# atharris/basilisk_env

Measured on NVIDIA B200. Metric: env decision-steps/sec, higher is better.
Workload: dtype f64

## Files before the change

basilisk_env_b200/csrc/leo_core.cuh:

```cuda
#pragma once
#include <math.h>
#include <stdint.h>
#include "leo_params.h"

#if defined(__CUDACC__)
#define LEO_HD __host__ __device__ __forceinline__
#define LEO_HD_NOINLINE static __host__ __device__ __noinline__
#else
#define LEO_HD inline
#define LEO_HD_NOINLINE static inline
#endif

#ifndef LEO_UNROLL_STAGES
#define LEO_UNROLL_STAGES 0
#endif

namespace leo {

struct V3 { double x, y, z; };
struct M3 { V3 a, b, c; };
LEO_HD V3 mk(double x, double y, double z) { V3 v; v.x = x; v.y = y; v.z = z; return v; }
LEO_HD V3 operator+(V3 p, V3 q) { return mk(p.x + q.x, p.y + q.y, p.z + q.z); }
LEO_HD V3 operator-(V3 p, V3 q) { return mk(p.x - q.x, p.y - q.y, p.z - q.z); }
LEO_HD V3 operator-(V3 p) { return mk(-p.x, -p.y, -p.z); }
// ... 767 lines not shown
        if (desat_quiet) {
            const int64_t cnt = I[(int64_t)I_DUMPCNT * stride + e];
            I[(int64_t)I_DUMPCNT * stride + e] = cnt <= 0 ? (int64_t)P.maxCounterValue : cnt - 1;
            I[(int64_t)I_DUMPPRIOR * stride + e] = now_ns;
            desat_ran = 4;
        } else {
            desat_ran = 1 | (fsw_desat<NRW>(P, S, I, stride, e, now_ns, ws) << 1);
        }
    }
    if (mask & LEO_TASK_MRP) {
        AttGuid g;
        g.sigma_BR = mld3(m, M_GUID); g.omega_BR_B = mld3(m, M_GUID + 3);
        g.omega_RN_B = mld3(m, M_GUID + 6); g.domega_RN_B = mld3(m, M_GUID + 9);
        V3 Lr = mrp_feedback(P, g);
        mst3(m, M_LR, Lr);
        g = att_tracking_error(ns, nw, ref);
        mst3(m, M_GUID, g.sigma_BR); mst3(m, M_GUID + 3, g.omega_BR_B);
        mst3(m, M_GUID + 6, g.omega_RN_B); mst3(m, M_GUID + 9, g.domega_RN_B);
        V3 mLr = -Lr;
#pragma unroll
        for (int i = 0; i < NRW; i++) mst(m, M_RWCMD + i, P.Umap[i][0] * mLr.x + P.Umap[i][1] * mLr.y + P.Umap[i][2] * mLr.z);
    }
    return desat_ran;
}

LEO_HD V3 add_cross(V3 p, V3 u, V3 v)
{
    return mk(fmad(u.y, v.z, fmad(-u.z, v.y, p.x)), fmad(u.z, v.x, fmad(-u.x, v.z, p.y)), fmad(u.x, v.y, fmad(-u.y, v.x, p.z)));
}
LEO_HD V3 sub_cross(V3 p, V3 u, V3 v)
{
    return mk(fmad(-u.y, v.z, fmad(u.z, v.y, p.x)), fmad(-u.z, v.x, fmad(u.x, v.z, p.y)), fmad(-u.x, v.y, fmad(u.y, v.x, p.z)));
}

LEO_HD V3 sun_accel(const LeoParams &P, V3 rs, V3 r)
{
    V3 d = r - rs;
    double is = rsq(dot(rs, rs)), id = rsq(dot(d, d));
    return rs * (-P.mu_sun * (is * is * is)) + d * (-P.mu_sun * (id * id * id));
}

LEO_HD V3 sun_window(const LeoParams &P, MBus m, const Dyn &x, double dt0, double h_first, int w, double dyn_s)
{
    const double half = 0.5 * (h_first + (double)(w - 1) * dyn_s);
    return sun_accel(P, mld3(m, M_SUNR) + mld3(m, M_SUNV) * (dt0 + half), x.r + x.v * half);
}

struct StageIn {
    V3 Lc;
    V3 gsun;
    V3 HB, tau_u;
    double rho, h;
    double dtp;
};

template <int J2, bool DIAG>
LEO_HD void eom(const LeoParams &P, const Dyn &x, Dyn &k, const StageIn &a, double ct, bool thr_on, MBus m)
{
    V3 g;
    {
        double ir = rsq(dot(x.r, x.r));
        double ir3 = ir * ir * ir;
        g = a.gsun + x.r * (-P.mu_c * ir3);
        if (J2 == 2) {
            const V3 D0 = mld3(m, M_PFIX) + mld3(m, M_PFIXD) * a.dtp;
            const V3 D1 = mld3(m, M_PFIX + 3) + mld3(m, M_PFIXD + 3) * a.dtp;
            const V3 D2 = mld3(m, M_PFIX + 6) + mld3(m, M_PFIXD + 6) * a.dtp;
            const V3 rp = mk(dot(D0, x.r), dot(D1, x.r), dot(D2, x.r));
            const double ip = rsq(dot(rp, rp)), ip2 = ip * ip, ip5 = ip2 * ip2 * ip;
            const V3 Mr = mk(P.gm2[0] * rp.x + P.gm2[3] * rp.y + P.gm2[4] * rp.z,
                             P.gm2[3] * rp.x + P.gm2[1] * rp.y + P.gm2[5] * rp.z,
                             P.gm2[4] * rp.x + P.gm2[5] * rp.y + P.gm2[2] * rp.z);
            const double q5 = -5. * dot(rp, Mr) * ip5 * ip2;
            const V3 gp = Mr * (2. * ip5) + rp * q5;
            g = g + D0 * gp.x + D1 * gp.y + D2 * gp.z;
        } else if (J2) {
            double ir2 = ir * ir, z2 = 5. * x.r.z * x.r.z * ir2, kk = -P.j2k * ir3 * ir2;
            g = g + mk(kk * x.r.x * (1. - z2), kk * x.r.y * (1. - z2), kk * x.r.z * (3. - z2));
        }
    }
    MrpRot R = mrp_rot(x.s);
    V3 vB = rot_BN(R, x.s, x.v);
    V3 Mp;
    double Sp;
    {
        double ax = fabs(vB.x), ay = fabs(vB.y), az = fabs(vB.z);
        Sp = P.dragKa[0] * ax + P.dragKa[1] * ay + P.dragKa[2] * az;
        if (!DIAG) Sp += P.dragKd[0] * vB.x + P.dragKd[1] * vB.y + P.dragKd[2] * vB.z;
        if (DIAG) {
            Mp = mk(P.dragMa[0][0] * ax + P.dragMd[0][0] * vB.x, P.dragMa[1][1] * ay + P.dragMd[1][1] * vB.y,
                    P.dragMa[2][2] * az + P.dragMd[2][2] * vB.z);
        } else {
            Mp = arr(P.dragMa[0]) * ax + arr(P.dragMa[1]) * ay + arr(P.dragMa[2]) * az
               + arr(P.dragMd[0]) * vB.x + arr(P.dragMd[1]) * vB.y + arr(P.dragMd[2]) * vB.z;
        }
    }
    const double mrho = -a.rho;
    k.v = g + x.v * (mrho * Sp);
    if (thr_on) k.v = k.v + rot_NB(R, x.s, mld3(m, M_FM));
    k.r = x.v;
    V3 rot = add_cross(a.Lc, Mp * mrho, vB);
    const V3 hw = a.HB + a.tau_u * ct;
    if (DIAG) {
        V3 h = mk(fmad(P.D[0], x.w.x, hw.x), fmad(P.D[4], x.w.y, hw.y), fmad(P.D[8], x.w.z, hw.z));
        rot = sub_cross(rot, x.w, h);
        k.w = mk(rot.x * P.Dinv[0], rot.y * P.Dinv[4], rot.z * P.Dinv[8]);
    } else {
        V3 h = mv9(P.D, x.w) + hw;
        rot = sub_cross(rot, x.w, h);
        k.w = mv9(P.Dinv, rot);
    }
    {
        double sw = dot(x.s, x.w);
        k.s = x.w * (0.25 * R.oms2) + cross(x.s, x.w) * 0.5 + x.s * (0.5 * sw);
    }
}

template <int J2, bool DIAG>
LEO_HD Dyn rk4_step(const LeoParams &P, const Dyn &x, const StageIn &a, bool thr_on, MBus m)
{
    const double h = a.h, hh = 0.5 * h, h6 = h * (1.0 / 6.0), h3 = h * (1.0 / 3.0);
    Dyn k, acc;
    k.r = k.v = k.s = k.w = acc.r = acc.v = acc.s = acc.w = mk(0., 0., 0.);
    double c = 0.;
#if LEO_UNROLL_STAGES == 2
#pragma unroll 2
#elif LEO_UNROLL_STAGES
#pragma unroll
#else
#pragma unroll 1
#endif
    for (int st = 0; st < 4; st++) {
        Dyn xs;
        xs.r = x.r + k.r * c; xs.v = x.v + k.v * c; xs.s = x.s + k.s * c; xs.w = x.w + k.w * c;
        eom<J2, DIAG>(P, xs, k, a, c, thr_on, m);
        const double wo = (st == 0 || st == 3) ? h6 : h3;
        acc.r = acc.r + k.r * wo; acc.v = acc.v + k.v * wo; acc.s = acc.s + k.s * wo; acc.w = acc.w + k.w * wo;
        c = (st == 2) ? h : hh;
    }
    Dyn xo;
    xo.r = x.r + acc.r; xo.v = x.v + acc.v; xo.s = x.s + acc.s; xo.w = x.w + acc.w;
    return xo;
}

struct SunDt { double d0, dm, d1; };
struct ThrEventOut { Dyn x; int factor, active; };
template <int J2, bool DIAG>
LEO_HD_NOINLINE ThrEventOut rk4_general(const LeoParams &P, const double *S, int64_t stride, int64_t e, MBus m, Dyn x,
                                        StageIn a, SunDt dts, double tBefore, double tauPrev, int thr_factor, int thr_active)
{
    const double h = a.h, hh = 0.5 * h, h6 = h * (1.0 / 6.0), h3 = h * (1.0 / 3.0);
    const V3 sun_r = mld3(m, M_SUNR), sun_v = mld3(m, M_SUNV), L_ext = mld3(m, M_LEXT);
    Dyn xs = x, xo = x, k;
    ThrCmd tc = {};
    if (thr_active) tc = thr_cmd_load(S, stride, e);
#pragma unroll 1
    for (int st = 0; st < 4; st++) {
        const double dt = (st == 0) ? dts.d0 : (st == 3 ? dts.d1 : dts.dm);
        const double ct = (st == 0) ? 0.0 : (st == 3 ? h : hh);
        a.gsun = sun_accel(P, sun_r + sun_v * dt, xs.r);
        a.dtp = dt;
        V3 Fm = mk(0., 0., 0.), Lx = L_ext;
        const bool thr_on = thr_active != 0;
        if (thr_on) {
            const double tau = t_add(tBefore, (st == 0) ? 0.0 : (st == 3 ? h : t_mul(h, 0.5)));
            ThrOut to = thr_stage(P, tc, tau, t_sub(tau, tauPrev), thr_factor);
            thr_factor = to.factor; thr_active = to.active;
            Fm = to.F * P.inv_mass; Lx = Lx + to.L;
            tauPrev = tau;
        }
        a.Lc = Lx - a.tau_u;
        mst3(m, M_FM, Fm);
        eom<J2, DIAG>(P, xs, k, a, ct, thr_on, m);
        const double wo = (st == 0 || st == 3) ? h6 : h3;
        const double cn = (st == 2) ? h : hh;
        xo.r = xo.r + k.r * wo; xo.v = xo.v + k.v * wo; xo.s = xo.s + k.s * wo; xo.w = xo.w + k.w * wo;
        if (st < 3) { xs.r = x.r + k.r * cn; xs.v = x.v + k.v * cn; xs.s = x.s + k.s * cn; xs.w = x.w + k.w * cn; }
    }
    ThrEventOut o;
    o.x = xo; o.factor = thr_factor; o.active = thr_active;
    return o;
}

struct ThrRefresh { V3 Lc, L_thr; double t_next; };
LEO_HD_NOINLINE ThrRefresh thr_refresh(const LeoParams &P, const double *S, int64_t stride, int64_t e, MBus m, int factor, V3 tau_u)
{
    ThrRefresh o;
    V3 F = mk(0., 0., 0.);
    o.L_thr = mk(0., 0., 0.); o.t_next = 1e300;
    double start = S[(int64_t)F_THRSTART * stride + e];
    for (int k = 0; k < LEO_NTHR; k++) {
        if (!((factor >> k) & 1)) continue;
        V3 f = arr(P.thr_dir[k]) * (P.thr_Fmax * 1.0);
        F = f + F;
        o.L_thr = cross(arr(P.thr_loc[k]), f) + o.L_thr;
        double t_off = t_add(S[(int64_t)(F_THRON + k) * stride + e], start);
        if (t_off < o.t_next) o.t_next = t_off;
    }
    mst3(m, M_FM, F * P.inv_mass);
    o.Lc = (mld3(m, M_LEXT) + o.L_thr) - tau_u;
    return o;
}

LEO_HD_NOINLINE SunDt sun_dt_wrapped(double prev_ns_d, double sun_ns_d, double tBefore, double prevTime, double h)
{
    SunDt o;
    uint64_t sun_ns = (uint64_t)sun_ns_d;
    uint64_t s0 = (uint64_t)t_add(prev_ns_d, t_div(t_sub(tBefore, prevTime), 1e-9));
    uint64_t sm = (uint64_t)t_add(prev_ns_d, t_div(t_sub(t_add(tBefore, t_mul(h, 0.5)), prevTime), 1e-9));
    uint64_t s1 = (uint64_t)t_add(prev_ns_d, t_div(t_sub(t_add(tBefore, h), prevTime), 1e-9));
    o.d0 = t_mul((double)(s0 - sun_ns), 1e-9);
    o.dm = t_mul((double)(sm - sun_ns), 1e-9);
    o.d1 = t_mul((double)(s1 - sun_ns), 1e-9);
    return o;
}

template <int NRW>
struct PostOut { double uJ[NRW]; V3 Lc, tau_u; int thr_active, quiet; };
template <int NRW>
LEO_HD void wheel_latch(const LeoParams &P, MBus m, const double (&W)[NRW], V3 L_thr, double (&uJ)[NRW], V3 &Lc, V3 &tau_u_out)
{
    V3 tau_u = mk(0., 0., 0.);
#pragma unroll
    for (int i = 0; i < NRW; i++) {
        double uc = mld(m, M_RWCMD + i);
        if (P.u_max[i] > 0.) { if (uc > P.u_max[i]) uc = P.u_max[i]; else if (uc < -P.u_max[i]) uc = -P.u_max[i]; }
        if (fabs(uc) < P.u_min[i]) uc = 0.0;
        if (fabs(W[i]) >= P.Om_max[i] && P.Om_max[i] > 0.0 && W[i] * uc >= 0.0) uc = 0.0;
        mst(m, M_U + i, uc);
        uJ[i] = uc * P.invJs[i];
        tau_u = tau_u + arr(P.gs[i]) * uc;
    }
    tau_u_out = tau_u;
    Lc = (mld3(m, M_LEXT) + L_thr) - tau_u;
}
template <int NRW>
LEO_HD_NOINLINE PostOut<NRW> post_tick_events(const LeoParams &P, double *S, int64_t *I, int64_t stride, int64_t e, MBus m,
                                              const double (&W)[NRW], V3 L_thr, int desat_ran, int64_t now_ns, int thr_factor)
{
    PostOut<NRW> o;
    wheel_latch<NRW>(P, m, W, L_thr, o.uJ, o.Lc, o.tau_u);
    o.thr_active = -1; o.quiet = 0;
    if (desat_ran & 1) {
        o.thr_active = thr_latch(P, S, I, stride, e, now_ns, thr_factor);
        o.quiet = (desat_ran & 2) && o.thr_active == 0;
    } else if (desat_ran & 4) {
        S[(int64_t)F_THRSTART * stride + e] = t_mul((double)now_ns, 1.0E-9);
        o.quiet = 1;
    }
    return o;
}

#define LEO_THR_MARGIN 1e-6

template <int NRW, bool DIAG>
LEO_HD void wheel_speeds(const LeoParams &P, V3 HB, const double (&C)[NRW], V3 w, double (&W)[NRW])
{
    if (DIAG) {
        W[0] = fmad(HB.x, P.invJs[0], -w.x); W[1] = fmad(HB.y, P.invJs[1], -w.y); W[2] = fmad(HB.z, P.invJs[2], -w.z);
    } else {
#pragma unroll
        for (int i = 0; i < NRW; i++) W[i] = C[i] - dot(arr(P.gs[i]), w);
    }
}

#if defined(__CUDACC__)
__constant__ double LEO_K[16] = {
    1.4426950408889634, 6755399441055744.0, -6.93147180369123816490e-01, -1.90821492927058770002e-10,
    1. / 6., 1. / 24., 1. / 120., 1. / 720., 1. / 5040., 1. / 40320., 1. / 362880., 1. / 3628800., 1. / 39916800.,
    1. / 479001600., 1. / 6227020800.,
    1e-9};
#endif
#if defined(__CUDA_ARCH__)
#define LEO_NANO2SEC LEO_K[15]
#else
#define LEO_NANO2SEC 1e-9
#endif
LEO_HD double exp_bounded(double x)
{
#ifdef __CUDA_ARCH__
    x = fmin(fmax(x, -700.0), 700.0);
    const double t = fma(x, LEO_K[0], LEO_K[1]);
    const int kk = __double2loint(t);
    const double kd = t - LEO_K[1];
    double r = fma(kd, LEO_K[2], x);
    r = fma(kd, LEO_K[3], r);
    const double r2 = r * r, r4 = r2 * r2, r8 = r4 * r4;
    const double a0 = r + 1.0, a1 = fma(r, LEO_K[4], 0.5), a2 = fma(r, LEO_K[6], LEO_K[5]), a3 = fma(r, LEO_K[8], LEO_K[7]);
    const double a4 = fma(r, LEO_K[10], LEO_K[9]), a5 = fma(r, LEO_K[12], LEO_K[11]);
    const double a6 = fma(r, LEO_K[14], LEO_K[13]);
    const double b0 = fma(a1, r2, a0), b1 = fma(a3, r2, a2), b2 = fma(a5, r2, a4);
    const double d0 = fma(b1, r4, b0), d1 = fma(a6, r4, b2);
    const double p = fma(d1, r8, d0);
    return __hiloint2double(__double2hiint(p) + (kk << 20), __double2loint(p));
#else
    return exp(x);
#endif
}

}
#include "leo_f32.cuh"
namespace leo {

template <int NRW, int J2, bool DIAG, bool F32 = false>
LEO_HD void leo_step_env(const LeoParams &P, double *__restrict__ S, int64_t *__restrict__ I, int64_t stride, int64_t e,
                         MBus m, int action, StepOut &out, const LeoParamsF &PF = LeoParamsF(), int chunk = 0, int n_chunks = 1)
{
#define SD(f) S[(int64_t)(f) * stride + e]
#define SI(f) I[(int64_t)(f) * stride + e]
    Dyn x;
    StageIn a;
    x.r = mk(SD(F_R), SD(F_R + 1), SD(F_R + 2));
    x.v = mk(SD(F_V), SD(F_V + 1), SD(F_V + 2));
    x.s = mk(SD(F_SIG), SD(F_SIG + 1), SD(F_SIG + 2));
    x.w = mk(SD(F_OMG), SD(F_OMG + 1), SD(F_OMG + 2));
    double C[NRW], uJ[NRW];
    a.tau_u = mk(0., 0., 0.); a.HB = mk(0., 0., 0.);
#pragma unroll
    for (int i = 0; i < NRW; i++) {
        const double u = SD(F_UCUR + i);
        mst(m, M_U + i, u);
        uJ[i] = u * P.invJs[i];
        C[i] = SD(F_WHL + i) + dot(arr(P.gs[i]), x.w);
        a.tau_u = a.tau_u + arr(P.gs[i]) * u;
        a.HB = a.HB + arr(P.gs[i]) * (P.Js[i] * C[i]);
    }
    for (int f = 0; f < LEO_M_MIRROR; f++) mst(m, f, SD(F_GUID + f));
    a.rho = SD(F_RHO);
    {
        const V3 L_ext = mk(SD(F_LDIST), SD(F_LDIST + 1), SD(F_LDIST + 2));
        mst3(m, M_LEXT, L_ext); mst3(m, M_FM, mk(0., 0., 0.));
        a.Lc = L_ext - a.tau_u;
    }
    mst3(m, M_LTHR, mk(0., 0., 0.));
    const int64_t tick = SI(I_TICK);
    int mask = (int)SI(I_MASK);
    int thr_factor = (int)SI(I_THRFACTOR), thr_active = (int)SI(I_THRACTIVE), rw_sat = (int)SI(I_RWSAT);
    int nswitch = 0;

    if (chunk > 0) {}
    else if (action == 0) mask = LEO_TASK_NADIR | LEO_TASK_MRP;
    else if (action == 1) mask = LEO_TASK_SUN | LEO_TASK_MRP;
    else if (action == 2) {
        mask = LEO_TASK_SUN | LEO_TASK_MRP | LEO_TASK_DESAT;
        SI(I_INITREQ) = 1;
        SI(I_DUMPPRIOR) = 0; SI(I_DUMPCNT) = 0; SI(I_LASTDH) = 0;
        for (int k = 0; k < LEO_NTHR; k++) SD(F_THRREM + k) = 0.0;
    }
    mst(m, M_TNEXT, -1.0);

    const bool first = tick < 0;
    const int tpf = P.ticks_per_fsw;
    const int ticks_step = tpf * P.fsw_per_step;
    const int ticks = ticks_step / n_chunks;
    const int64_t n_base = (first ? 0 : tick) + 1;
    const int64_t n_step0 = ((n_base - 1) / ticks_step) * ticks_step;
    const int64_t n_end = n_step0 + ticks_step;
    const double dyn_d = (double)P.dyn_ns;
    double sun_d = (double)(n_step0 * P.dyn_ns);
    sun_latch_to_bus(P, m, n_step0 * P.dyn_ns);
    if (J2 == 2) pfix_latch_to_bus(P, m, n_step0 * P.dyn_ns);
    a.dtp = 0.;
    V3f sunr_f = mkf(0.f, 0.f, 0.f), sunv_f = mkf(0.f, 0.f, 0.f);
    float ecf[6] = {0.f, 0.f, 0.f, 0.f, 0.f, 0.f};
    if (F32) {
        sunr_f = tof(mld3(m, M_SUNR)); sunv_f = tof(mld3(m, M_SUNV));
#pragma unroll
        for (int q = 0; q < 6; q++) ecf[q] = (float)mld(m, M_ECL + q);
    }
    const int j0 = first ? -1 : 0;
    int phase = (int)((n_base + j0) % tpf);
    double now_d = (double)((n_base + j0) * P.dyn_ns);
    int desat_ran = 0, desat_quiet = 0;
    double charge = SD(F_E), shadow = SD(F_SHADOW);
    double newTime = t_mul(now_d, LEO_NANO2SEC);
    double prevTime = j0 < 0 ? 0.0 : t_mul(now_d - dyn_d, 1e-9);
    double h = t_sub(newTime, prevTime);
    double dtsm = t_mul((j0 < 0 ? 0.0 : now_d - dyn_d) - sun_d, LEO_NANO2SEC) + 0.5 * h;
    const double dyn_s = t_mul(dyn_d, LEO_NANO2SEC);
    if (!F32) a.gsun = sun_window(P, m, x, dtsm - 0.5 * h, h, tpf - phase, dyn_s);

#pragma unroll 1
    for (int j = j0; j < ticks; j++) {
        bool wrapped = false;
        if (LEO_RARE(phase == 0)) {
            const int64_t n = n_base + j;
            double W[NRW];
            wheel_speeds<NRW, DIAG>(P, a.HB, C, x.w, W);
#ifndef LEO_EXP_NOFSW
            desat_ran = fsw_pass<NRW>(P, S, I, stride, e, m, mask, n, n * P.dyn_ns, x, W, (int64_t)sun_d, desat_quiet);
            rw_sat |= 2;
#endif
            if (n > 0 && n == n_end) {
                sun_d = now_d; sun_latch_to_bus(P, m, n * P.dyn_ns); wrapped = true;
                if (J2 == 2) pfix_latch_to_bus(P, m, n * P.dyn_ns);
                if (F32) {
                    sunr_f = tof(mld3(m, M_SUNR)); sunv_f = tof(mld3(m, M_SUNV));
#pragma unroll
                    for (int q = 0; q < 6; q++) ecf[q] = (float)mld(m, M_ECL + q);
                }
            }
            if (!F32) a.gsun = sun_window(P, m, x, t_mul((j < 0 ? 0.0 : now_d - dyn_d) - sun_d, LEO_NANO2SEC), h, tpf, dyn_s);
        }
        a.h = h;
        if (LEO_RARE(wrapped || (thr_active && !(newTime + LEO_THR_MARGIN <= mld(m, M_TNEXT))))) {
            const double prev_d = j < 0 ? 0.0 : now_d - dyn_d;
            const double tBefore = t_sub(newTime, h);
            SunDt dts;
            dts.d0 = t_mul(prev_d - sun_d, 1e-9); dts.dm = dts.d0 + 0.5 * h; dts.d1 = dts.d0 + h;
            if (wrapped) dts = sun_dt_wrapped(prev_d, sun_d, tBefore, prevTime, h);
            double tauPrev = 0.0;
            if (j >= 0) {
                const double ppT = (n_base + j > 1) ? t_mul(prev_d - dyn_d, 1e-9) : 0.0;
                const double ph = t_sub(prevTime, ppT);
                tauPrev = t_add(t_sub(prevTime, ph), ph);
            }
            ThrEventOut o = rk4_general<J2, DIAG>(P, S, stride, e, m, x, a, dts, tBefore, tauPrev, thr_factor, thr_active);
            x = o.x; thr_factor = o.factor; thr_active = o.active;
            ThrRefresh th = thr_refresh(P, S, stride, e, m, thr_active ? thr_factor : 0, a.tau_u);
            a.Lc = th.Lc; mst3(m, M_LTHR, th.L_thr); mst(m, M_TNEXT, th.t_next);
        } else if (F32) {
            StageInF af;
            af.h = (float)h; af.rho = (float)a.rho;
            af.Lc = tof(a.Lc); af.HB = tof(a.HB); af.tau_u = tof(a.tau_u);
            af.gsun = sun_accelf(PF, sunr_f + sunv_f * (float)dtsm, tof(x.r) + tof(x.v) * (0.5f * af.h));
            const bool thr_on = thr_active != 0;
            x = rk4_step_mixed<(J2 != 0), DIAG>(PF, x, af, thr_on, thr_on ? tof(mld3(m, M_FM)) : mkf(0.f, 0.f, 0.f));
        } else {
            if (J2 == 2) a.dtp = dtsm;
            x = rk4_step<J2, DIAG>(P, x, a, thr_active != 0, m);
        }
        a.HB = a.HB + a.tau_u * h;
        if (!DIAG) {
#pragma unroll
            for (int i = 0; i < NRW; i++) C[i] = fmad(uJ[i], h, C[i]);
        }
        {
            const double s2 = dot(x.s, x.s);
            const bool sw = s2 > 1.0000000000000002;
            const double f = -frcp(sw ? s2 : 1.0);
            x.s = mk(sw ? x.s.x * f : x.s.x, sw ? x.s.y * f : x.s.y, sw ? x.s.z * f : x.s.z);
            nswitch += sw ? 1 : 0;
        }
        double r2 = 0., ir = 0., id = 0., rdh = 0., pgeo = 0.;
        bool penumbra = false;
        float shf = 0.f, panel_f = 0.f;
        V3f xr_f = mkf(0.f, 0.f, 0.f);
        if (F32) {
            xr_f = tof(x.r);
            const float r2f = dot(xr_f, xr_f);
            a.rho = (double)(PF.rho0 * expf(-(r2f * rsqf(r2f) - PF.Rp_atmo) * PF.inv_H));
            const V3f r_SBf = sunr_f - xr_f;
            const float d2f = dot(r_SBf, r_SBf), idf = rsqf(d2f);
            shf = eclipse_coref(PF, ecf, sunr_f, xr_f, r2f, d2f);
            penumbra = shf < 0.f;
            const V3f sf = tof(x.s);
            MrpRotF R = mrp_rotf(sf);
            V3f n_N = rot_NBf(R, sf, arrf(PF.nHat_B));
            float proj = dot(n_N, r_SBf) * idf;
            if (proj < 0.f) proj = 0.f;
            panel_f = PF.panel_coef * proj * (idf * idf);
        } else {
            r2 = dot(x.r, x.r); ir = rsq(r2);
            a.rho = P.rho0 * exp_bounded(-(r2 * ir - P.Rp_atmo) * P.inv_H);
        }
        double W[NRW];
        wheel_speeds<NRW, DIAG>(P, a.HB, C, x.w, W);
        int lim = 0;
#pragma unroll
        for (int i = 0; i < NRW; i++) lim |= (fabs(W[i]) >= P.Om_max[i] && P.Om_max[i] > 0.0) ? 1 : 0;
#ifndef LEO_EXP_NOENV
        if (!F32) {
            const V3 sun_r = mld3(m, M_SUNR);
            const V3 r_SB = sun_r - x.r;
            const double d2 = dot(r_SB, r_SB);
            id = rsq(d2);
            const double ec[6] = {mld(m, M_ECL), mld(m, M_ECL + 1), mld(m, M_ECL + 2), mld(m, M_ECL + 3), mld(m, M_ECL + 4), mld(m, M_ECL + 5)};
            shadow = eclipse_cones(P, ec, sun_r, x.r, r2, d2, penumbra);
            rdh = dot(x.r, r_SB);
            MrpRot R = mrp_rot(x.s);
            V3 n_N = rot_NB(R, x.s, arr(P.nHat_B));
            double proj = dot(n_N, r_SB) * id;
            if (proj < 0.) proj = 0.;
            pgeo = P.panel_coef * proj * (id * id);
        }
#endif
        const double h_this = h;
        now_d += dyn_d;
        phase = (phase + 1 == tpf) ? 0 : phase + 1;
        prevTime = newTime;
        newTime = t_mul(now_d, LEO_NANO2SEC);
        h = t_sub(newTime, prevTime);
        dtsm = t_mul((now_d - dyn_d) - sun_d, LEO_NANO2SEC) + 0.5 * h;
        if (LEO_RARE(rw_sat | lim | desat_ran)) {
            PostOut<NRW> po = post_tick_events<NRW>(P, S, I, stride, e, m, W, mld3(m, M_LTHR), desat_ran, (int64_t)(now_d - dyn_d), thr_factor);
#pragma unroll
            for (int i = 0; i < NRW; i++) uJ[i] = po.uJ[i];
            a.Lc = po.Lc; a.tau_u = po.tau_u;
            rw_sat = lim;
            if (po.thr_active >= 0) { thr_active = po.thr_active; mst(m, M_TNEXT, -1.0); }
            if (desat_ran) desat_quiet = po.quiet;
            desat_ran = 0;
        }
        if (LEO_RARE(penumbra)) {
            if (F32) {
                const V3 sun_r = mld3(m, M_SUNR);
                const V3 r_SB = sun_r - x.r;
                const double r2d = dot(x.r, x.r), d2 = dot(r_SB, r_SB);
                const double ec[6] = {mld(m, M_ECL), mld(m, M_ECL + 1), mld(m, M_ECL + 2), mld(m, M_ECL + 3), mld(m, M_ECL + 4), mld(m, M_ECL + 5)};
                shadow = eclipse_core(P, ec, sun_r, x.r, r2d, rsq(r2d), r_SB, d2, rsq(d2));
                shf = (float)shadow;
            } else {
#ifdef LEO_LITERAL_ECLIPSE
                shadow = penumbra_literal(P, mld3(m, M_SUNR), x.r);
#else
                shadow = penumbra_fraction(P, ir, id, rdh);
#endif
            }
        } else if (F32) {
            shadow = (double)shf;
        }
        {
            const double panel = F32 ? (double)(panel_f * shf) : pgeo * shadow;
            double E = charge + (panel + P.sink_power) * h_this;
            if (E > P.capacity) E = P.capacity;
            if (E < 0.) E = 0.;
            charge = j >= 0 ? E : charge;
        }
    }
    for (int f = 0; f < LEO_M_MIRROR; f++) SD(F_GUID + f) = mld(m, f);
    double W[NRW];
    wheel_speeds<NRW, DIAG>(P, a.HB, C, x.w, W);
    if (chunk + 1 < n_chunks) {
        SD(F_R) = x.r.x; SD(F_R + 1) = x.r.y; SD(F_R + 2) = x.r.z;
        SD(F_V) = x.v.x; SD(F_V + 1) = x.v.y; SD(F_V + 2) = x.v.z;
        SD(F_SIG) = x.s.x; SD(F_SIG + 1) = x.s.y; SD(F_SIG + 2) = x.s.z;
        SD(F_OMG) = x.w.x; SD(F_OMG + 1) = x.w.y; SD(F_OMG + 2) = x.w.z;
#pragma unroll
        for (int i = 0; i < NRW; i++) { SD(F_WHL + i) = W[i]; SD(F_UCUR + i) = mld(m, M_U + i); }
        SD(F_RHO) = a.rho; SD(F_E) = charge; SD(F_SHADOW) = shadow;
        SI(I_TICK) = n_base - 1 + ticks; SI(I_MASK) = mask; SI(I_SWITCH) = SI(I_SWITCH) + nswitch;
        SI(I_THRFACTOR) = thr_factor; SI(I_THRACTIVE) = thr_active; SI(I_RWSAT) = rw_sat;
        out.done = 0; out.reason = 0; out.reward = 0.;
        return;
    }
    double ob0 = norm(mld3(m, M_GUID));
    double ob1 = norm(x.w);
    double wn = 0.;
#pragma unroll
    for (int i = 0; i < NRW; i++) wn += W[i] * W[i];
    const double E = charge;
    double ob2 = sqrt(wn), ob3 = E / 3600., ob4 = shadow;
    int sim_over = norm(x.r) < P.decay_radius;
    int64_t curr_step = SI(I_STEP);
    int over = (int)SI(I_OVER), reason = 0;
    if (curr_step >= P.max_length) { over = 1; reason |= 1; }
    double reward = 0.;
    if (action == 0) reward = fabs(P.reward_mult / (1. + ob0 * ob0));
    double ret = SD(F_EPRET) + reward;
    SD(F_OBS) = ob0; SD(F_OBS + 1) = ob1; SD(F_OBS + 2) = ob2; SD(F_OBS + 3) = ob3; SD(F_OBS + 4) = ob4;
    ob2 = ob2 / P.wheel_limit;
    ob3 = ob3 / P.power_max;
    if (ob2 > 1.) { over = 1; reward -= P.failure_penalty; ret -= P.failure_penalty; reason |= 2; }
    if (ob3 == 0.) { over = 1; reward -= P.failure_penalty; ret -= P.failure_penalty; reason |= 4; }
    if (sim_over) { over = 1; reason |= 8; }
    out.ob[0] = ob0; out.ob[1] = ob1; out.ob[2] = ob2; out.ob[3] = ob3; out.ob[4] = ob4;
    out.reward = reward; out.done = over; out.reason = reason;

    SD(F_R) = x.r.x; SD(F_R + 1) = x.r.y; SD(F_R + 2) = x.r.z;
    SD(F_V) = x.v.x; SD(F_V + 1) = x.v.y; SD(F_V + 2) = x.v.z;
    SD(F_SIG) = x.s.x; SD(F_SIG + 1) = x.s.y; SD(F_SIG + 2) = x.s.z;
    SD(F_OMG) = x.w.x; SD(F_OMG + 1) = x.w.y; SD(F_OMG + 2) = x.w.z;
#pragma unroll
    for (int i = 0; i < NRW; i++) { SD(F_WHL + i) = W[i]; SD(F_UCUR + i) = mld(m, M_U + i); }
    SD(F_RHO) = a.rho; SD(F_E) = E; SD(F_SHADOW) = shadow; SD(F_EPRET) = ret;
    SI(I_TICK) = n_end; SI(I_STEP) = curr_step + 1; SI(I_MASK) = mask; SI(I_SWITCH) = SI(I_SWITCH) + nswitch;
    SI(I_THRFACTOR) = thr_factor; SI(I_THRACTIVE) = thr_active; SI(I_OVER) = over; SI(I_RWSAT) = rw_sat;
#undef SD
#undef SI
}

}
```

Measured before the change: 10.03 million.

## Restructure tick loop into warp-uniform inner fast path with deferred rare events

Splits the per-tick loop into an outer loop per FSW phase window and an inner tight loop that runs only the common RK4, environment and battery path. Rare events (wheel saturation, penumbra, MRP switch, latch) break out of the inner loop by warp-wide vote and are handled afterwards. Thruster-window exits are also decided warp-wide. The aim is to cut divergent branches and per-tick overhead inside the hot loop. In exchange it adds warp-vote synchronisation, and one lane's event forces the whole warp out of the fast path.

```diff
diff --git a/basilisk_env_b200/csrc/leo_core.cuh b/basilisk_env_b200/csrc/leo_core.cuh
--- a/basilisk_env_b200/csrc/leo_core.cuh
+++ b/basilisk_env_b200/csrc/leo_core.cuh
@@ -1093,6 +1093,23 @@
 #include "leo_f32.cuh"
 namespace leo {
 
+LEO_HD bool leo_warp_any(bool c)
+{
+#ifdef __CUDA_ARCH__
+    return __any_sync(__activemask(), c);
+#else
+    return c;
+#endif
+}
+
+LEO_HD double battery(const LeoParams &P, double charge, double panel, double h, bool tick0)
+{
+    double E = charge + (panel + P.sink_power) * h;
+    if (E > P.capacity) E = P.capacity;
+    if (E < 0.) E = 0.;
+    return tick0 ? charge : E;
+}
+
 template <int NRW, int J2, bool DIAG, bool F32 = false>
 LEO_HD void leo_step_env(const LeoParams &P, double *__restrict__ S, int64_t *__restrict__ I, int64_t stride, int64_t e,
                          MBus m, int action, StepOut &out, const LeoParamsF &PF = LeoParamsF(), int chunk = 0, int n_chunks = 1)
@@ -1171,8 +1188,9 @@
     const double dyn_s = t_mul(dyn_d, LEO_NANO2SEC);
     if (!F32) a.gsun = sun_window(P, m, x, dtsm - 0.5 * h, h, tpf - phase, dyn_s);
 
+    int j = j0;
 #pragma unroll 1
-    for (int j = j0; j < ticks; j++) {
+    while (j < ticks) {
         bool wrapped = false;
         if (LEO_RARE(phase == 0)) {
             const int64_t n = n_base + j;
@@ -1193,8 +1211,9 @@
             }
             if (!F32) a.gsun = sun_window(P, m, x, t_mul((j < 0 ? 0.0 : now_d - dyn_d) - sun_d, LEO_NANO2SEC), h, tpf, dyn_s);
         }
-        a.h = h;
-        if (LEO_RARE(wrapped || (thr_active && !(newTime + LEO_THR_MARGIN <= mld(m, M_TNEXT))))) {
+        const bool general = wrapped || (thr_active && !(newTime + LEO_THR_MARGIN <= mld(m, M_TNEXT)));
+        if (LEO_RARE(general)) {
+            a.h = h;
             const double prev_d = j < 0 ? 0.0 : now_d - dyn_d;
             const double tBefore = t_sub(newTime, h);
             SunDt dts;
@@ -1210,81 +1229,105 @@
             x = o.x; thr_factor = o.factor; thr_active = o.active;
             ThrRefresh th = thr_refresh(P, S, stride, e, m, thr_active ? thr_factor : 0, a.tau_u);
             a.Lc = th.Lc; mst3(m, M_LTHR, th.L_thr); mst(m, M_TNEXT, th.t_next);
-        } else if (F32) {
-            StageInF af;
-            af.h = (float)h; af.rho = (float)a.rho;
-            af.Lc = tof(a.Lc); af.HB = tof(a.HB); af.tau_u = tof(a.tau_u);
-            af.gsun = sun_accelf(PF, sunr_f + sunv_f * (float)dtsm, tof(x.r) + tof(x.v) * (0.5f * af.h));
-            const bool thr_on = thr_active != 0;
-            x = rk4_step_mixed<(J2 != 0), DIAG>(PF, x, af, thr_on, thr_on ? tof(mld3(m, M_FM)) : mkf(0.f, 0.f, 0.f));
-        } else {
-            if (J2 == 2) a.dtp = dtsm;
-            x = rk4_step<J2, DIAG>(P, x, a, thr_active != 0, m);
-        }
-        a.HB = a.HB + a.tau_u * h;
-        if (!DIAG) {
-#pragma unroll
-            for (int i = 0; i < NRW; i++) C[i] = fmad(uJ[i], h, C[i]);
-        }
-        {
-            const double s2 = dot(x.s, x.s);
-            const bool sw = s2 > 1.0000000000000002;
-            const double f = -frcp(sw ? s2 : 1.0);
-            x.s = mk(sw ? x.s.x * f : x.s.x, sw ? x.s.y * f : x.s.y, sw ? x.s.z * f : x.s.z);
-            nswitch += sw ? 1 : 0;
-        }
-        double r2 = 0., ir = 0., id = 0., rdh = 0., pgeo = 0.;
-        bool penumbra = false;
+        }
+        const int j_entry = j, j_stop = (j + tpf - phase < ticks) ? j + tpf - phase : ticks;
+        int latch_due = rw_sat | desat_ran;
+        double W[NRW];
+        double ir = 0., id = 0., rdh = 0., pgeo = 0., h_this = 0.;
+        bool penumbra = false, event = false, mid_tick = false, mrp_sw = false;
+        int lim = 0;
         float shf = 0.f, panel_f = 0.f;
-        V3f xr_f = mkf(0.f, 0.f, 0.f);
-        if (F32) {
-            xr_f = tof(x.r);
-            const float r2f = dot(xr_f, xr_f);
-            a.rho = (double)(PF.rho0 * expf(-(r2f * rsqf(r2f) - PF.Rp_atmo) * PF.inv_H));
-            const V3f r_SBf = sunr_f - xr_f;
-            const float d2f = dot(r_SBf, r_SBf), idf = rsqf(d2f);
-            shf = eclipse_coref(PF, ecf, sunr_f, xr_f, r2f, d2f);
-            penumbra = shf < 0.f;
-            const V3f sf = tof(x.s);
-            MrpRotF R = mrp_rotf(sf);
-            V3f n_N = rot_NBf(R, sf, arrf(PF.nHat_B));
-            float proj = dot(n_N, r_SBf) * idf;
-            if (proj < 0.f) proj = 0.f;
-            panel_f = PF.panel_coef * proj * (idf * idf);
-        } else {
-            r2 = dot(x.r, x.r); ir = rsq(r2);
-            a.rho = P.rho0 * exp_bounded(-(r2 * ir - P.Rp_atmo) * P.inv_H);
-        }
-        double W[NRW];
-        wheel_speeds<NRW, DIAG>(P, a.HB, C, x.w, W);
-        int lim = 0;
-#pragma unroll
-        for (int i = 0; i < NRW; i++) lim |= (fabs(W[i]) >= P.Om_max[i] && P.Om_max[i] > 0.0) ? 1 : 0;
+        bool integrated = general;
+#pragma unroll 1
+        for (;;) {
+            if (!integrated) {
+                a.h = h;
+                if (F32) {
+                    StageInF af;
+                    af.h = (float)h; af.rho = (float)a.rho;
+                    af.Lc = tof(a.Lc); af.HB = tof(a.HB); af.tau_u = tof(a.tau_u);
+                    af.gsun = sun_accelf(PF, sunr_f + sunv_f * (float)dtsm, tof(x.r) + tof(x.v) * (0.5f * af.h));
+                    const bool thr_on = thr_active != 0;
+                    x = rk4_step_mixed<(J2 != 0), DIAG>(PF, x, af, thr_on, thr_on ? tof(mld3(m, M_FM)) : mkf(0.f, 0.f, 0.f));
+                } else {
+                    if (J2 == 2) a.dtp = dtsm;
+                    x = rk4_step<J2, DIAG>(P, x, a, thr_active != 0, m);
+                }
+            }
+            integrated = false;
+            a.HB = a.HB + a.tau_u * h;
+            if (!DIAG) {
+#pragma unroll
+                for (int i = 0; i < NRW; i++) C[i] = fmad(uJ[i], h, C[i]);
+            }
+            {
+                const double s2 = dot(x.s, x.s);
+                const bool sw = s2 > 1.0000000000000002;
+                const double f = -frcp(sw ? s2 : 1.0);
+                x.s = mk(sw ? x.s.x * f : x.s.x, sw ? x.s.y * f : x.s.y, sw ? x.s.z * f : x.s.z);
+                mrp_sw = sw;
+            }
+            double r2 = 0.;
+            penumbra = false;
+            V3f xr_f = mkf(0.f, 0.f, 0.f);
+            if (F32) {
+                xr_f = tof(x.r);
+                const float r2f = dot(xr_f, xr_f);
+                a.rho = (double)(PF.rho0 * expf(-(r2f * rsqf(r2f) - PF.Rp_atmo) * PF.inv_H));
+                const V3f r_SBf = sunr_f - xr_f;
+                const float d2f = dot(r_SBf, r_SBf), idf = rsqf(d2f);
+                shf = eclipse_coref(PF, ecf, sunr_f, xr_f, r2f, d2f);
+                penumbra = shf < 0.f;
+                const V3f sf = tof(x.s);
+                MrpRotF R = mrp_rotf(sf);
+                V3f n_N = rot_NBf(R, sf, arrf(PF.nHat_B));
+                float proj = dot(n_N, r_SBf) * idf;
+                if (proj < 0.f) proj = 0.f;
+                panel_f = PF.panel_coef * proj * (idf * idf);
+            } else {
+                r2 = dot(x.r, x.r); ir = rsq(r2);
+                a.rho = P.rho0 * exp_bounded(-(r2 * ir - P.Rp_atmo) * P.inv_H);
+            }
+            wheel_speeds<NRW, DIAG>(P, a.HB, C, x.w, W);
+            lim = 0;
+#pragma unroll
+            for (int i = 0; i < NRW; i++) lim |= (fabs(W[i]) >= P.Om_max[i] && P.Om_max[i] > 0.0) ? 1 : 0;
 #ifndef LEO_EXP_NOENV
-        if (!F32) {
-            const V3 sun_r = mld3(m, M_SUNR);
-            const V3 r_SB = sun_r - x.r;
-            const double d2 = dot(r_SB, r_SB);
-            id = rsq(d2);
-            const double ec[6] = {mld(m, M_ECL), mld(m, M_ECL + 1), mld(m, M_ECL + 2), mld(m, M_ECL + 3), mld(m, M_ECL + 4), mld(m, M_ECL + 5)};
-            shadow = eclipse_cones(P, ec, sun_r, x.r, r2, d2, penumbra);
-            rdh = dot(x.r, r_SB);
-            MrpRot R = mrp_rot(x.s);
-            V3 n_N = rot_NB(R, x.s, arr(P.nHat_B));
-            double proj = dot(n_N, r_SB) * id;
-            if (proj < 0.) proj = 0.;
-            pgeo = P.panel_coef * proj * (id * id);
-        }
-#endif
-        const double h_this = h;
-        now_d += dyn_d;
-        phase = (phase + 1 == tpf) ? 0 : phase + 1;
-        prevTime = newTime;
-        newTime = t_mul(now_d, LEO_NANO2SEC);
-        h = t_sub(newTime, prevTime);
-        dtsm = t_mul((now_d - dyn_d) - sun_d, LEO_NANO2SEC) + 0.5 * h;
-        if (LEO_RARE(rw_sat | lim | desat_ran)) {
-            PostOut<NRW> po = post_tick_events<NRW>(P, S, I, stride, e, m, W, mld3(m, M_LTHR), desat_ran, (int64_t)(now_d - dyn_d), thr_factor);
+            if (!F32) {
+                const V3 sun_r = mld3(m, M_SUNR);
+                const V3 r_SB = sun_r - x.r;
+                const double d2 = dot(r_SB, r_SB);
+                id = rsq(d2);
+                const double ec[6] = {mld(m, M_ECL), mld(m, M_ECL + 1), mld(m, M_ECL + 2), mld(m, M_ECL + 3), mld(m, M_ECL + 4), mld(m, M_ECL + 5)};
+                shadow = eclipse_cones(P, ec, sun_r, x.r, r2, d2, penumbra);
+                rdh = dot(x.r, r_SB);
+                MrpRot R = mrp_rot(x.s);
+                V3 n_N = rot_NB(R, x.s, arr(P.nHat_B));
+                double proj = dot(n_N, r_SB) * id;
+                if (proj < 0.) proj = 0.;
+                pgeo = P.panel_coef * proj * (id * id);
+            }
+#endif
+            h_this = h;
+            now_d += dyn_d;
+            prevTime = newTime;
+            newTime = t_mul(now_d, LEO_NANO2SEC);
+            h = t_sub(newTime, prevTime);
+            dtsm = t_mul((now_d - dyn_d) - sun_d, LEO_NANO2SEC) + 0.5 * h;
+            event = (latch_due | lim) || penumbra || mrp_sw;
+            if (LEO_RARE(leo_warp_any(event))) { mid_tick = true; break; }
+            latch_due = 0;
+            if (F32) shadow = (double)shf;
+            charge = battery(P, charge, F32 ? (double)(panel_f * shf) : pgeo * shadow, h_this, j < 0);
+            j++;
+            if (leo_warp_any(j >= j_stop || (thr_active && !(newTime + LEO_THR_MARGIN <= mld(m, M_TNEXT))))) break;
+        }
+        if (event && mrp_sw) nswitch++;
+        if (event && (rw_sat | lim | desat_ran)) {
+            double Wl[NRW];
+#pragma unroll
+            for (int i = 0; i < NRW; i++) Wl[i] = W[i];
+            PostOut<NRW> po = post_tick_events<NRW>(P, S, I, stride, e, m, Wl, mld3(m, M_LTHR), desat_ran, (int64_t)(now_d - dyn_d), thr_factor);
 #pragma unroll
             for (int i = 0; i < NRW; i++) uJ[i] = po.uJ[i];
             a.Lc = po.Lc; a.tau_u = po.tau_u;
@@ -1293,7 +1336,7 @@
             if (desat_ran) desat_quiet = po.quiet;
             desat_ran = 0;
         }
-        if (LEO_RARE(penumbra)) {
+        if (event && penumbra) {
             if (F32) {
                 const V3 sun_r = mld3(m, M_SUNR);
                 const V3 r_SB = sun_r - x.r;
@@ -1308,16 +1351,15 @@
                 shadow = penumbra_fraction(P, ir, id, rdh);
 #endif
             }
-        } else if (F32) {
+        } else if (mid_tick && F32) {
             shadow = (double)shf;
         }
-        {
-            const double panel = F32 ? (double)(panel_f * shf) : pgeo * shadow;
-            double E = charge + (panel + P.sink_power) * h_this;
-            if (E > P.capacity) E = P.capacity;
-            if (E < 0.) E = 0.;
-            charge = j >= 0 ? E : charge;
-        }
+        if (mid_tick) {
+            charge = battery(P, charge, F32 ? (double)(panel_f * shf) : pgeo * shadow, h_this, j < 0);
+            j++;
+        }
+        phase += j - j_entry;
+        if (phase == tpf) phase = 0;
     }
     for (int f = 0; f < LEO_M_MIRROR; f++) SD(F_GUID + f) = mld(m, f);
     double W[NRW];
```

Result: faster. 10.26 million, median of 6 (+2.3%).
